# wenbowen123/iros20-6d-pose-tracking

Measured on NVIDIA H100. Metric: rgbd_pair_frames_per_sec, higher is better.
Workload: dtype bf16x3 (bf16 hi/lo split operands, 3 products/MAC, fp32 accumulate)

## Files before the change

### iros20-6d-pose-tracking_b200/csrc/conv_wgmma.cu

```cuda
#include "conv_common.h"
#include "launch.h"
#include "ptx.cuh"
#include "storage.cuh"
#include <algorithm>

namespace se3tn {
namespace {

constexpr int kThreads2 = 384;
constexpr int kPoolPitch = 68;
constexpr int kPoolStageBytes = 121 * kPoolPitch * 4;
constexpr int kPoolStageAlloc = (kPoolStageBytes + 1023) & ~1023;
constexpr int kWgRowBytes = 64 * kChunkBytes;

template <int KIND> struct KTab;
template <> struct KTab<KIND_S1> {
    static constexpr int NU = 3;
    static constexpr int kAUnit = 19 * 1024;
    __host__ __device__ static constexpr int ntaps(int) { return 3; }
    __host__ __device__ static constexpr int wtap(int u, int k) { return k * 3 + u; }
    __host__ __device__ static constexpr int amap(int) { return 0; }
    __host__ __device__ static constexpr int c1(int u) { return u - 1; }
    __host__ __device__ static constexpr int c2(int) { return -1; }
    __host__ __device__ static constexpr int rows(int) { return 11 * 13; }
};
template <> struct KTab<KIND_S2> {
    static constexpr int NU = 6;
    static constexpr int kAUnit = 19 * 1024;
    __host__ __device__ static constexpr int ntaps(int u) { return (u & 1) ? 2 : 1; }
    __host__ __device__ static constexpr int wtap(int u, int k) { return (u & 1) ? (k == 0 ? (u >> 1) : 6 + (u >> 1)) : 3 + (u >> 1); }
    __host__ __device__ static constexpr int amap(int u) { return (u & 1) * 2 + ((u >> 1) == 1 ? 0 : 1); }
    __host__ __device__ static constexpr int c1(int u) { return (u >> 1) == 0 ? -1 : 0; }
    __host__ __device__ static constexpr int c2(int u) { return (u & 1) ? -1 : 0; }
    __host__ __device__ static constexpr int rows(int u) { return (u & 1) ? 11 * 12 : 11 * 11; }
};
template <> struct KTab<KIND_STEM> {
    static constexpr int NU = 2;
    static constexpr int kAUnit = 21 * 1024;
    __host__ __device__ static constexpr int ntaps(int u) { return u == 0 ? 4 : 3; }
    __host__ __device__ static constexpr int wtap(int u, int k) { return 2 * k + u; }
    __host__ __device__ static constexpr int amap(int u) { return u; }
    __host__ __device__ static constexpr int c1(int) { return 0; }
    __host__ __device__ static constexpr int c2(int) { return 0; }
    __host__ __device__ static constexpr int rows(int u) { return u == 0 ? 11 * 14 : 11 * 13; }
};
constexpr int kRowShift = 11;

__device__ __forceinline__ float selu_fast(float x) {
    constexpr float kAlpha = 1.6732632423543772f, kScale = 1.0507009873554805f;
    return x > 0.f ? kScale * x : (kScale * kAlpha) * (__expf(x) - 1.f);
}
__device__ __forceinline__ float act_apply(float x, int act) {
    return act == ACT_RELU ? fmaxf(x, 0.f) : (act == ACT_SELU ? selu_fast(x) : x);
}

__device__ __forceinline__ unsigned long long gtimer() { unsigned long long t; asm volatile("mov.u64 %0, %%globaltimer;" : "=l"(t)); return t; }
__device__ __forceinline__ void trace_stamp(unsigned long long* tr, int slot) { if (tr) tr[blockIdx.x * 8 + slot] = gtimer(); }
__device__ __forceinline__ void trace_exit(unsigned long long* tr) {
    if (!tr) return;
    unsigned smid; asm volatile("mov.u32 %0, %%smid;" : "=r"(smid));
    tr[blockIdx.x * 8 + 7] = (gtimer() & ~0xffull) | (smid & 0xff);
}
__device__ __forceinline__ void tile_stamp(unsigned long long* tt, int tile, int k) {
    if (tt && tile < SE3TN_TRACE_TILES) tt[tile * 4 + k] = k == 3 ? (gtimer() & ~0xffull) | (blockIdx.x & 0xff) : gtimer();
}

using ptx::desc_lo;
using ptx::mk_desc;

__device__ __forceinline__ float (&acc_lo32(float (&d)[64]))[32] { return *reinterpret_cast<float (*)[32]>(&d[0]); }

struct Consumer {
    int ct, cg, cw, ew, lane, R, m;
    __device__ __forceinline__ Consumer() {
        ct = static_cast<int>(threadIdx.x) - 128; cg = ct >> 7; ew = ct >> 5; cw = ew & 3; lane = ct & 31; R = lane >> 2; m = lane & 3;
    }
    __device__ __forceinline__ bool leader() const { return (ct & 127) == 0; }
    __device__ __forceinline__ int row(int half, int h) const { return 64 * half + 16 * cw + R + 8 * h; }
};

constexpr int kProducerRegs = 40;
constexpr int kConsumerRegs = 232;
constexpr int kTurnBar = 1;
constexpr int kStageBar = 3;
constexpr int kEpiBar = 5;

template <int N> struct Ring {
    uint32_t phase = 0;
    int stage = 0;
    __device__ __forceinline__ void next() { if (++stage == N) { stage = 0; phase ^= 1; } }
    __device__ __forceinline__ void skip(int n) {
        stage += n;
        phase ^= static_cast<uint32_t>(stage / N) & 1u;
        stage %= N;
    }
    __device__ __forceinline__ uint32_t producer_parity() const { return phase ^ 1; }
    __device__ __forceinline__ uint32_t consumer_parity() const { return phase; }
};

struct Turn {
    int base, g;
    __device__ __forceinline__ void begin() const { if (g == 1) ptx::bar_arrive(base, 256); }
    __device__ __forceinline__ void wait() const { ptx::bar_sync(base + g, 256); }
    __device__ __forceinline__ void pass() const { ptx::bar_arrive(base + (g ^ 1), 256); }
    __device__ __forceinline__ bool mine(int t) const { return (t & 1) == g; }
    __device__ __forceinline__ void end(int turns) const { if (mine(turns)) wait(); }
};

template <int KIND, int N>
__device__ __forceinline__ void load_a_units(const LayerDesc& L, int ox, int oy, int cbase, int img, int c0, int c1,
                                             uint8_t* sA, uint64_t* a_full, uint64_t* a_empty, Ring<N>& ring)
{
    using KT = KTab<KIND>;
    for (int ch = c0; ch < c1; ++ch) {
#pragma unroll
        for (int u = 0; u < KT::NU; ++u) {
            ptx::mbar_wait(&a_empty[ring.stage], ring.producer_parity());
            ptx::mbar_arrive_expect_tx(&a_full[ring.stage], static_cast<uint32_t>(KT::rows(u)) * kChunkBytes);
            ptx::tma_load_4d(sA + ring.stage * KT::kAUnit, &L.amap[KT::amap(u)], &a_full[ring.stage],
                             cbase + ch * 32, ox + KT::c1(u), oy + KT::c2(u), img);
            ring.next();
        }
    }
}

template <int PREC, int N>
__device__ __forceinline__ void mma_chunk(float (&acc)[N / 2], uint32_t a_lo, uint32_t b_lo, uint32_t fresh) {
#pragma unroll
    for (int kk = 0; kk < 4; ++kk) {
        const uint64_t a = mk_desc(a_lo + 2 * kk), b = mk_desc(b_lo + 2 * kk);
        const uint32_t f = fresh | (kk ? 1u : 0u);
        if constexpr (PREC == SE3TN_PREC_TF32) {
            if constexpr (N == 64) ptx::wgmma_tf32_n64(acc, a, b, f); else ptx::wgmma_tf32_n128(acc, a, b, f);
        } else if constexpr (PREC == SE3TN_PREC_FP8) {
            static_assert(N == 128, "e4m3 MMAs only in the trunk");
            ptx::wgmma_e4m3_n128(acc, a, b, f);
        } else if constexpr (PREC == SE3TN_PREC_FP16) {
            if constexpr (N == 64) ptx::wgmma_f16_n64(acc, a, b, f); else ptx::wgmma_f16_n128(acc, a, b, f);
        } else {
            if constexpr (N == 64) ptx::wgmma_bf16_n64(acc, a, b, f); else ptx::wgmma_bf16_n128(acc, a, b, f);
        }
    }
}

template <int KIND, int PREC> struct RCfg {
    static constexpr bool POOL = (KIND == KIND_STEM);
    static constexpr int BN = 64;
    static constexpr int kStack = ((POOL ? stem_input_prec(PREC) : PREC) == SE3TN_PREC_BF16X3) ? 2 : 1;
    static constexpr int kBTile = BN * kStack * kChunkBytes;
    static constexpr int kAStages = POOL ? (PREC == SE3TN_PREC_TF32 ? 4 : 3) : (prec_2byte(PREC) ? 6 : 4);
    static constexpr int kPoolBufs = POOL ? (PREC == SE3TN_PREC_TF32 ? 2 : 1) : 0;
    static constexpr int kAcc = BN * kStack / 2;
    static constexpr int kMaxWTiles = POOL ? 7 : ((PREC == SE3TN_PREC_TF32) ? 18 : 9);
    static constexpr int kSmem = kAStages * KTab<KIND>::kAUnit + kMaxWTiles * kBTile + kPoolBufs * kPoolStageAlloc + 1024 + 512;
    static_assert(kSmem <= 232448, "shared memory budget");
};

template <int KIND, int PREC>
__device__ __forceinline__ void resident_mma_unit(float (&acc)[RCfg<KIND, PREC>::kAcc], uint32_t a_unit_lo, const uint8_t* sB,
                                                  int u, int ch, int tiles_per_tap, uint32_t& fresh)
{
    using C = RCfg<KIND, PREC>;
    using KT = KTab<KIND>;
#pragma unroll
    for (int k = 0; k < 4; ++k) {
        if (k >= KT::ntaps(u)) break;
        const uint32_t a_lo = a_unit_lo + k * kRowShift * (kChunkBytes >> 4);
        uint32_t b_lo;
        if (C::kStack == 2) b_lo = desc_lo(sB + KT::wtap(u, k) * C::kBTile) + ch * 4;
        else                b_lo = desc_lo(sB + (KT::wtap(u, k) * tiles_per_tap + ch) * C::kBTile);
        if constexpr (C::kStack == 2 && !C::POOL) {
#pragma unroll
            for (int sl = 0; sl < 2; ++sl) {
                ptx::wgmma_bf16_n128(acc, mk_desc(a_lo + 2 * sl), mk_desc(b_lo + 2 * sl), fresh | (sl ? 1u : 0u));
                ptx::wgmma_bf16_n64(acc_lo32(acc), mk_desc(a_lo + 4 + 2 * sl), mk_desc(b_lo + 2 * sl), 1u);
            }
        } else {
            mma_chunk<C::POOL ? stem_input_prec(PREC) : PREC, C::BN * C::kStack>(acc, a_lo, b_lo, fresh);
        }
        fresh = 1u;
    }
}

template <int KIND, int PREC, bool PP>
__global__ void __launch_bounds__(kThreads2, 1)
conv_resident_kernel(const __grid_constant__ ResidentParams p)
{
    constexpr int AP = resident_prec(PREC);
    static_assert(PREC != SE3TN_PREC_FP8 || KIND == KIND_S1, "e4m3 output: the 64-channel layers only");
    using C = RCfg<KIND, AP>;
    using KT = KTab<KIND>;
    constexpr bool POOL = C::POOL;
    constexpr int NH = PP ? 2 : 1;
    constexpr bool kShareStage = PP && C::kPoolBufs == 1;
    extern __shared__ uint8_t smem_raw[];
    uint8_t* smem = reinterpret_cast<uint8_t*>((reinterpret_cast<uintptr_t>(smem_raw) + 1023) & ~uintptr_t(1023));
    const LayerDesc& L = p.L;
    const int chunks = L.chunks;
    const int tiles_per_tap = (C::kStack == 2) ? 1 : chunks;
    uint8_t* sA = smem;
    uint8_t* sB = sA + C::kAStages * KT::kAUnit;
    uint8_t* sP = sB + C::kMaxWTiles * C::kBTile;
    uint64_t* bars = reinterpret_cast<uint64_t*>(sP + C::kPoolBufs * kPoolStageAlloc);
    uint64_t* a_full = bars;
    uint64_t* a_empty = a_full + C::kAStages;
    uint64_t* b_full = a_empty + C::kAStages;
    uint64_t* b_empty = b_full + KT::NU;

    ptx::grid_dep_launch();
    if (threadIdx.x == 0) trace_stamp(p.trace, 0);
    const int warp = threadIdx.x >> 5;
    const int lane = threadIdx.x & 31;
    const int tiles_img = L.tiles_x * L.tiles_y;
    const int w_begin = static_cast<int>(static_cast<long long>(blockIdx.x) * p.m_tiles / gridDim.x);
    const int w_end = static_cast<int>(static_cast<long long>(blockIdx.x + 1) * p.m_tiles / gridDim.x);
    auto img_of = [&](int tile) -> int { return p.img_first + tile / tiles_img; };
    auto wid_of = [&](int tile) -> int { return p.img_wid ? p.img_wid[img_of(tile)] : -1; };

    if (threadIdx.x == 0) {
        for (int s = 0; s < C::kAStages; ++s) { ptx::mbar_init(&a_full[s], 1); ptx::mbar_init(&a_empty[s], PP ? 1 : 2); }
        for (int u = 0; u < KT::NU; ++u) ptx::mbar_init(&b_full[u], 1);
        ptx::mbar_init(&b_empty[0], 2);
        ptx::fence_barrier_init();
        ptx::fence_proxy_async();
    }
    __syncthreads();
    if (threadIdx.x == 0) trace_stamp(p.trace, 1);

    if (warp < 4) {
        ptx::setmaxnreg_dec<kProducerRegs>();
        if (warp == 0) {
            if (lane == 0) {
                ptx::grid_dep_wait();
                Ring<C::kAStages> ring;
                for (int tile = w_begin; tile < w_end; ++tile) {
                    const int n0 = img_of(tile), r = tile % tiles_img;
                    const int ty = r / L.tiles_x, tx = r - ty * L.tiles_x;
                    load_a_units<KIND>(L, tx * p.step_x + p.off_x, ty * p.step_y + p.off_y, 0, n0, 0, chunks, sA, a_full, a_empty, ring);
                }
            }
        } else if (warp == 1) {
            if (lane == 0) {
                int cur = -2; uint32_t gen = 0;
                for (int tile = w_begin; tile < w_end; ++tile) {
                    const int wid = wid_of(tile);
                    if (wid == cur) continue;
                    if (gen) ptx::mbar_wait(&b_empty[0], (gen - 1) & 1);
                    const CUtensorMap* bm = wid < 0 ? &L.bmap : p.gbmaps + wid * kLayersPerSet + L.li;
#pragma unroll
                    for (int u = 0; u < KT::NU; ++u) {
                        ptx::mbar_arrive_expect_tx(&b_full[u], static_cast<uint32_t>(KT::ntaps(u) * tiles_per_tap) * C::kBTile);
#pragma unroll
                        for (int k = 0; k < KT::ntaps(u); ++k)
                            for (int c = 0; c < tiles_per_tap; ++c) {
                                const int wt = KT::wtap(u, k) * tiles_per_tap + c;
                                ptx::tma_load_2d(sB + wt * C::kBTile, bm, &b_full[u], wt * 32, 0);
                            }
                    }
                    cur = wid; ++gen;
                }
            }
        }
    } else {
        ptx::setmaxnreg_inc<kConsumerRegs>();
        ptx::grid_dep_wait();
        using S = Storage<AP>;
        const Consumer cs;
        const bool stamp = threadIdx.x == 128;
        const bool tstamp = cs.leader() && (PP || cs.cg == 0);
        constexpr int kEpiThreads = PP ? 128 : 256;
        const int et = PP ? (cs.ct & 127) : cs.ct;
        auto half_of = [&](int hf) { return PP ? hf : cs.cg; };
        Ring<C::kAStages> a_ring;
        int w_cur = -2; uint32_t w_gen = 0;
        const Turn turn{kTurnBar, cs.cg}, stage_turn{kStageBar, cs.cg};
        if constexpr (PP) {
            turn.begin();
            if constexpr (kShareStage) stage_turn.begin();
        }
        int it = 0;
        for (int tile = w_begin; tile < w_end; ++tile, ++it) {
            const int wid = wid_of(tile);
            const bool new_w = (wid != w_cur);
            const bool w_last = tile + 1 < w_end && wid_of(tile + 1) != wid;
            if (PP && !turn.mine(it)) {
                a_ring.skip(chunks * KT::NU);
                if (new_w) {
#pragma unroll
                    for (int u = 0; u < KT::NU; ++u) ptx::mbar_wait(&b_full[u], w_gen & 1);
                    w_cur = wid; ++w_gen;
                }
                if (w_last && cs.leader()) ptx::mbar_arrive(&b_empty[0]);
                continue;
            }
            const int n0 = img_of(tile), r = tile % tiles_img;
            const int ty = r / L.tiles_x, tx = r - ty * L.tiles_x;

            constexpr int kPreRes = (PP && C::kStack == 2) ? 1 : NH;
            size_t rpix[NH][2]; bool rvalid[NH][2]; Raw<AP, 8> rres[NH][2][2];
            auto load_res = [&](int hf) {
#pragma unroll
                for (int h = 0; h < 2; ++h) {
                    const int rw = cs.row(half_of(hf), h);
                    const int py = rw / 11, px = rw - py * 11;
                    const int y = ty * 11 + py, x = tx * 11 + px;
                    rvalid[hf][h] = (rw < 121) && (y < L.Ho) && (x < L.Wo);
                    rpix[hf][h] = (static_cast<size_t>(n0) * L.Ho + y) * L.Wo + x;
#pragma unroll
                    for (int b = 0; b < 2; ++b) {
                        rres[hf][h][b] = Raw<AP, 8>{};
                        if (L.res && rvalid[hf][h]) {
                            const uint8_t* rp = L.res + S::addr(rpix[hf][h], L.res_c, 32 * b + 8 * cs.m);
#pragma unroll
                            for (int q = 0; q < Raw<AP, 8>::kPieces; ++q) rres[hf][h][b].set(q, __ldg(Raw<AP, 8>::at(rp, q)));
                        }
                    }
                }
            };
            if constexpr (!POOL) {
#pragma unroll
                for (int hf = 0; hf < kPreRes; ++hf) load_res(hf);
            }
            float4 pb4 = make_float4(0.f, 0.f, 0.f, 0.f);
            if constexpr (POOL) pb4 = __ldg(reinterpret_cast<const float4*>((p.img_wid ? p.gbias[p.img_wid[n0] * kLayersPerSet + L.li] : L.bias) + (et & 15) * 4));

            float acc[NH][C::kAcc];
#pragma unroll
            for (int hf = 0; hf < NH; ++hf)
#pragma unroll
                for (int i = 0; i < C::kAcc; ++i) acc[hf][i] = 0.f;
            if constexpr (PP) turn.wait();
            uint32_t fresh = 0;
            int pend = -1;
            for (int ch = 0; ch < chunks; ++ch) {
#pragma unroll
                for (int u = 0; u < KT::NU; ++u) {
                    if (new_w && ch == 0) {
                        ptx::mbar_wait(&b_full[u], w_gen & 1);
                        if (it == 0 && u == 0 && stamp) trace_stamp(p.trace, 2);
                    }
                    ptx::mbar_wait(&a_full[a_ring.stage], a_ring.consumer_parity());
                    if (ch == 0 && u == 0) {
                        if (it == 0 && stamp) trace_stamp(p.trace, 3);
                        if (tstamp) tile_stamp(p.tile_trace, tile, 0);
                    }
                    ptx::wgmma_fence();
                    const uint32_t a_unit_lo = desc_lo(sA + a_ring.stage * KT::kAUnit);
#pragma unroll
                    for (int hf = 0; hf < NH; ++hf) {
                        uint32_t f = fresh;
                        resident_mma_unit<KIND, AP>(acc[hf], a_unit_lo + half_of(hf) * (kWgRowBytes >> 4), sB, u, ch, tiles_per_tap, f);
                    }
                    fresh = 1u;
                    ptx::wgmma_commit();
                    ptx::wgmma_wait<1>();
                    if (pend >= 0 && cs.leader()) ptx::mbar_arrive(&a_empty[pend]);
                    pend = a_ring.stage;
                    a_ring.next();
                }
            }
            if constexpr (PP) turn.pass();
            ptx::wgmma_wait<0>();
#pragma unroll
            for (int hf = 0; hf < NH; ++hf) ptx::wgmma_reg_fence(acc[hf]);
            if (tstamp) tile_stamp(p.tile_trace, tile, 1);
            if (cs.leader()) {
                ptx::mbar_arrive(&a_empty[pend]);
                if (w_last) ptx::mbar_arrive(&b_empty[0]);
            }
            if (new_w) { w_cur = wid; ++w_gen; }
            if (it == 0 && stamp) trace_stamp(p.trace, 5);
            if (tstamp) tile_stamp(p.tile_trace, tile, 2);

            if constexpr (!POOL) {
                float inv_out = 1.f;
                if constexpr (PREC == SE3TN_PREC_FP8) inv_out = 1.f / __ldg((p.img_wid ? p.gfp8[p.img_wid[n0]] : p.fp8) + L.q_out);
#pragma unroll
                for (int hf = 0; hf < NH; ++hf) {
                    if (hf >= kPreRes) load_res(hf);
#pragma unroll
                    for (int b = 0; b < 2; ++b) {
                        const int ch0 = 32 * b + 8 * cs.m;
                        const float* bias_base = (p.img_wid ? p.gbias[p.img_wid[n0] * kLayersPerSet + L.li] : L.bias) + ch0;
                        const float4 bA = __ldg(reinterpret_cast<const float4*>(bias_base)), bB = __ldg(reinterpret_cast<const float4*>(bias_base + 4));
                        const float bias8[8] = {bA.x, bA.y, bA.z, bA.w, bB.x, bB.y, bB.z, bB.w};
#pragma unroll
                        for (int h = 0; h < 2; ++h) {
                            if (!rvalid[hf][h]) continue;
                            float v[8];
#pragma unroll
                            for (int jj = 0; jj < 4; ++jj)
#pragma unroll
                                for (int e = 0; e < 2; ++e) {
                                    const int ri = 16 * b + 4 * jj + 2 * h + e;
                                    float a = acc[hf][ri];
                                    if constexpr (C::kStack == 2) a += acc[hf][32 + ri];
                                    v[2 * jj + e] = a + bias8[2 * jj + e];
                                }
                            if (L.res) {
                                float r[8];
                                S::decode(rres[hf][h][b], r);
#pragma unroll
                                for (int e = 0; e < 8; ++e) v[e] += r[e];
                            }
#pragma unroll
                            for (int e = 0; e < 8; ++e) v[e] = act_apply(v[e], L.act);
                            if constexpr (PREC == SE3TN_PREC_FP8) {
                                using S8 = Storage<SE3TN_PREC_FP8>;
#pragma unroll
                                for (int e = 0; e < 8; ++e) v[e] *= inv_out;
                                S8::encode(v).store(L.out + S8::addr(rpix[hf][h], L.out_c, L.out_coff + ch0));
                            } else {
                                S::encode(v).store(L.out + S::addr(rpix[hf][h], L.out_c, L.out_coff + ch0));
                            }
                        }
                    }
                }
            } else {
                float* stage = reinterpret_cast<float*>(sP + (C::kPoolBufs == 2 ? (it & 1) : 0) * kPoolStageAlloc);
                if constexpr (kShareStage) stage_turn.wait();
                else if constexpr (PP) ptx::bar_sync(kEpiBar + cs.cg, 128);
#pragma unroll
                for (int hf = 0; hf < NH; ++hf)
#pragma unroll
                    for (int h = 0; h < 2; ++h) {
                        const int rw = cs.row(half_of(hf), h);
                        if (rw >= 121) continue;
                        const int cy_l = rw / 11, cx_l = rw - cy_l * 11;
                        const int cy = ty * p.step_y + p.off_y + cy_l, cx = tx * p.step_x + p.off_x + cx_l;
                        const bool cvalid = cy >= 0 && cy < 88 && cx >= 0 && cx < 88;
                        float* srow = stage + rw * kPoolPitch + 2 * cs.m;
                        const float ninf = -3.0e38f;
#pragma unroll
                        for (int j = 0; j < 8; ++j) {
                            float a0 = acc[hf][4 * j + 2 * h], a1 = acc[hf][4 * j + 2 * h + 1];
                            if constexpr (C::kStack == 2) { a0 += acc[hf][32 + 4 * j + 2 * h]; a1 += acc[hf][32 + 4 * j + 2 * h + 1]; }
                            *reinterpret_cast<float2*>(srow + 8 * j) = cvalid ? make_float2(a0, a1) : make_float2(ninf, ninf);
                        }
                    }
                ptx::bar_sync(PP ? kEpiBar + cs.cg : kEpiBar, kEpiThreads);

                for (int v = et; v < 400; v += kEpiThreads) {
                    const int pp = v >> 4, c4 = (v & 15) * 4;
                    const int ppy = pp / 5, ppx = pp - ppy * 5;
                    const int oy = ty * 5 + ppy, ox = tx * 5 + ppx;
                    if (oy >= L.Ho || ox >= L.Wo) continue;
                    float4 mx = make_float4(-3.0e38f, -3.0e38f, -3.0e38f, -3.0e38f);
#pragma unroll
                    for (int dy = 0; dy < 3; ++dy)
#pragma unroll
                        for (int dx = 0; dx < 3; ++dx) {
                            const float4 s4 = *reinterpret_cast<const float4*>(stage + ((2 * ppy + dy) * 11 + 2 * ppx + dx) * kPoolPitch + c4);
                            mx.x = fmaxf(mx.x, s4.x); mx.y = fmaxf(mx.y, s4.y); mx.z = fmaxf(mx.z, s4.z); mx.w = fmaxf(mx.w, s4.w);
                        }
                    const float v4[4] = {selu_fast(mx.x + pb4.x), selu_fast(mx.y + pb4.y), selu_fast(mx.z + pb4.z), selu_fast(mx.w + pb4.w)};
                    S::encode(v4).store(L.out + S::addr((static_cast<size_t>(n0) * L.Ho + oy) * L.Wo + ox, L.out_c, L.out_coff + c4));
                }
                if constexpr (kShareStage) stage_turn.pass();
                else if constexpr (!PP) { if (C::kPoolBufs == 1) ptx::bar_sync(kEpiBar, 256); }
            }
            if (tstamp) tile_stamp(p.tile_trace, tile, 3);
        }
        if constexpr (PP) {
            turn.end(it);
            if constexpr (kShareStage) stage_turn.end(it);
        }
        if (stamp) { trace_stamp(p.trace, 4); trace_stamp(p.trace, 6); }
    }

    __syncthreads();
    if (threadIdx.x == 0) trace_exit(p.trace);
}

template <int PREC> struct TCfg {
    static constexpr int BN = 128;
    static constexpr int kAcc = BN / 2;
    static constexpr int kAStages = 3;
    static constexpr int kBStages = 6;
    static constexpr int kBTile = BN * kChunkBytes;
    static constexpr int kEpiPitch = 36;
    static constexpr int kEpiWarpBytes = 16 * kEpiPitch * 4 + 128;
    static constexpr int kEpiBytes = 8 * kEpiWarpBytes;
    static constexpr int kSched = 4;
    static constexpr int kAUnit = KTab<KIND_S1>::kAUnit;
    static_assert(kAUnit == KTab<KIND_S2>::kAUnit, "A ring stage size");
    static constexpr int kSmem = kAStages * kAUnit + kBStages * kBTile + ((kEpiBytes + 1023) & ~1023) + 1024 + 512;
    static_assert(kSmem <= 232448, "shared memory budget");
};
constexpr int kTaps3 = 9;

struct UnitCoord { int l, img, tx, ty, n_tile, grp, c0, c1, piece, gidx; };
__device__ __forceinline__ void unit_stamp(const TrunkParams& p, int u, int k) {
    if (p.trace && u < 2048) p.trace[256 * 8 + u * 5 + k] = k == 4 ? (gtimer() & ~0xffull) | (blockIdx.x & 0xff) : gtimer();
}

__device__ __forceinline__ int unit_layer(const TrunkParams& p, int u) {
    int l = 0;
#pragma unroll
    for (int i = 1; i < kTrunkMaxLayers; ++i) if (i < p.n_layers && u >= p.layer[i].unit_base) l = i;
    return l;
}

__device__ __forceinline__ UnitCoord decode_unit(const TrunkParams& p, int u) {
    UnitCoord c;
    c.l = unit_layer(p, u);
    const LayerDesc& L = p.layer[c.l];
    int local = u - L.unit_base;
    c.piece = 0; c.c0 = 0; c.c1 = L.chunks;
    if (p.ksplit > 1) {
        c.piece = local % p.ksplit; local /= p.ksplit;
        c.c0 = c.piece * L.chunks / p.ksplit; c.c1 = (c.piece + 1) * L.chunks / p.ksplit;
    }
    c.gidx = L.base_unit0 + local;
    const int im = local / L.units_per_image;
    int r = local - im * L.units_per_image;
    c.img = p.img_first + im;
    c.n_tile = r % L.n_tiles; r /= L.n_tiles;
    c.grp = r % L.groups; r /= L.groups;
    c.ty = r / L.tiles_x; c.tx = r - c.ty * L.tiles_x;
    return c;
}

template <int KIND, int PREC>
__device__ __forceinline__ void trunk_load_weights(const LayerDesc& L, const CUtensorMap* bm, const UnitCoord& c, uint8_t* sB,
                                                   uint64_t* b_full, uint64_t* b_empty, Ring<TCfg<PREC>::kBStages>& ring)
{
    using KT = KTab<KIND>;
    using C = TCfg<PREC>;
    const int wrow = c.grp * L.cout + c.n_tile * C::BN;
    for (int ch = c.c0; ch < c.c1; ++ch) {
#pragma unroll
        for (int u = 0; u < KT::NU; ++u) {
#pragma unroll
            for (int k = 0; k < KT::ntaps(u); ++k) {
                ptx::mbar_wait(&b_empty[ring.stage], ring.producer_parity());
                ptx::mbar_arrive_expect_tx(&b_full[ring.stage], C::kBTile);
                ptx::tma_load_2d(sB + ring.stage * C::kBTile, bm, &b_full[ring.stage], KT::wtap(u, k) * L.cin_words + ch * 32, wrow);
                ring.next();
            }
        }
    }
}

template <int KIND, int PREC>
__device__ __forceinline__ void trunk_mma_unit(float (&acc)[2][TCfg<PREC>::kAcc], const Consumer& cs, const Turn& turn, int chunks,
                                               uint8_t* sA, uint8_t* sB, uint64_t* a_full, uint64_t* a_empty, uint64_t* b_full,
                                               uint64_t* b_empty, Ring<TCfg<PREC>::kAStages>& a_ring, Ring<TCfg<PREC>::kBStages>& b_ring,
                                               unsigned long long* trace, bool first_unit, unsigned long long* ustamp)
{
    using KT = KTab<KIND>;
    using C = TCfg<PREC>;
    const bool stamp = cs.leader();
    uint32_t fresh = 0;
    int pend_b = -1, pend_a = -1;
    turn.wait();
    for (int ch = 0; ch < chunks; ++ch) {
#pragma unroll
        for (int u = 0; u < KT::NU; ++u) {
            ptx::mbar_wait(&a_full[a_ring.stage], a_ring.consumer_parity());
            if (first_unit && ch == 0 && u == 0 && stamp) trace_stamp(trace, 3);
            if (ustamp && ch == 0 && u == 0 && stamp) *ustamp = gtimer();
            const uint32_t a_unit_lo = desc_lo(sA + a_ring.stage * C::kAUnit);
#pragma unroll
            for (int k = 0; k < KT::ntaps(u); ++k) {
                ptx::mbar_wait(&b_full[b_ring.stage], b_ring.consumer_parity());
                if (first_unit && ch == 0 && u == 0 && k == 0 && stamp) trace_stamp(trace, 2);
                const uint32_t b_lo = desc_lo(sB + b_ring.stage * C::kBTile);
                ptx::wgmma_fence();
#pragma unroll
                for (int hf = 0; hf < 2; ++hf) {
                    const uint32_t a_lo = a_unit_lo + hf * (kWgRowBytes >> 4) + k * kRowShift * (kChunkBytes >> 4);
                    if constexpr (PREC == SE3TN_PREC_BF16X3) {
                        constexpr int AO[6] = {0, 2, 4, 6, 0, 2};
                        constexpr int BO[6] = {0, 2, 0, 2, 4, 6};
#pragma unroll
                        for (int i = 0; i < 6; ++i)
                            ptx::wgmma_bf16_n128(acc[hf], mk_desc(a_lo + AO[i]), mk_desc(b_lo + BO[i]), fresh | (i ? 1u : 0u));
                    } else {
                        mma_chunk<PREC, C::BN>(acc[hf], a_lo, b_lo, fresh);
                    }
                }
                ptx::wgmma_commit();
                ptx::wgmma_wait<1>();
                if (cs.leader()) {
                    if (pend_b >= 0) ptx::mbar_arrive(&b_empty[pend_b]);
                    if (pend_a >= 0) ptx::mbar_arrive(&a_empty[pend_a]);
                }
                pend_b = b_ring.stage;
                pend_a = (k + 1 == KT::ntaps(u)) ? a_ring.stage : -1;
                fresh = 1u;
                b_ring.next();
            }
            a_ring.next();
        }
    }
    turn.pass();
    ptx::wgmma_wait<0>();
    ptx::wgmma_reg_fence(acc[0]);
    ptx::wgmma_reg_fence(acc[1]);
    if (cs.leader()) {
        if (pend_b >= 0) ptx::mbar_arrive(&b_empty[pend_b]);
        if (pend_a >= 0) ptx::mbar_arrive(&a_empty[pend_a]);
    }
}

template <int PREC>
__global__ void __launch_bounds__(kThreads2, 1)
conv_trunk_kernel(const __grid_constant__ TrunkParams p)
{
    using C = TCfg<PREC>;
    constexpr int BN = C::BN;
    extern __shared__ uint8_t smem_raw[];
    uint8_t* smem = reinterpret_cast<uint8_t*>((reinterpret_cast<uintptr_t>(smem_raw) + 1023) & ~uintptr_t(1023));
    uint8_t* sA = smem;
    uint8_t* sB = sA + C::kAStages * C::kAUnit;
    uint8_t* sT = sB + C::kBStages * C::kBTile;
    uint64_t* bars = reinterpret_cast<uint64_t*>(sT + ((C::kEpiBytes + 1023) & ~1023));
    uint64_t* a_full = bars;
    uint64_t* a_empty = a_full + C::kAStages;
// ... 353 lines not shown
```

### iros20-6d-pose-tracking_b200/csrc/ptx.cuh

```cuda
#pragma once
#include <cstdint>
#include <cuda.h>

namespace ptx {

__device__ __forceinline__ uint32_t smem_u32(const void* p) {
    return static_cast<uint32_t>(__cvta_generic_to_shared(p));
}

__device__ __forceinline__ bool elect_one() {
    uint32_t pred = 0;
    asm volatile(
        "{\n\t.reg .pred P;\n\t"
        "elect.sync _|P, 0xffffffff;\n\t"
        "selp.u32 %0, 1, 0, P;\n\t}\n"
        : "=r"(pred));
    return pred != 0;
}

__device__ __forceinline__ int ld_acquire_gpu(const int* p) {
    int v;
    asm volatile("ld.acquire.gpu.global.s32 %0, [%1];" : "=r"(v) : "l"(p) : "memory");
    return v;
}
__device__ __forceinline__ void st_release_gpu(int* p, int v) {
    asm volatile("st.release.gpu.global.s32 [%0], %1;" :: "l"(p), "r"(v) : "memory");
}
__device__ __forceinline__ void grid_dep_launch() { asm volatile("griddepcontrol.launch_dependents;" ::: "memory"); }
__device__ __forceinline__ void grid_dep_wait()   { asm volatile("griddepcontrol.wait;" ::: "memory"); }

template <int N> __device__ __forceinline__ void setmaxnreg_dec() { asm volatile("setmaxnreg.dec.sync.aligned.u32 %0;" ::"n"(N)); }
template <int N> __device__ __forceinline__ void setmaxnreg_inc() { asm volatile("setmaxnreg.inc.sync.aligned.u32 %0;" ::"n"(N)); }
__device__ __forceinline__ void bar_sync(int id, int n)   { asm volatile("bar.sync %0, %1;" ::"r"(id), "r"(n) : "memory"); }
__device__ __forceinline__ void bar_arrive(int id, int n) { asm volatile("bar.arrive %0, %1;" ::"r"(id), "r"(n) : "memory"); }

__device__ __forceinline__ void mbar_init(uint64_t* bar, uint32_t count) {
    asm volatile("mbarrier.init.shared::cta.b64 [%0], %1;" ::"r"(smem_u32(bar)), "r"(count));
}
__device__ __forceinline__ void fence_barrier_init() {
    asm volatile("fence.mbarrier_init.release.cluster;" ::: "memory");
}
__device__ __forceinline__ void fence_proxy_async() {
    asm volatile("fence.proxy.async.shared::cta;" ::: "memory");
}
__device__ __forceinline__ void fence_proxy_async_all() {
    asm volatile("fence.proxy.async;" ::: "memory");
}
__device__ __forceinline__ void mbar_arrive_expect_tx(uint64_t* bar, uint32_t bytes) {
    asm volatile("mbarrier.arrive.expect_tx.shared::cta.b64 _, [%0], %1;"
                 ::"r"(smem_u32(bar)), "r"(bytes) : "memory");
}
__device__ __forceinline__ void mbar_arrive(uint64_t* bar) {
    asm volatile("mbarrier.arrive.shared::cta.b64 _, [%0];" ::"r"(smem_u32(bar)) : "memory");
}
__device__ __forceinline__ bool mbar_try_wait(uint64_t* bar, uint32_t parity) {
    uint32_t ok;
    asm volatile(
        "{\n\t.reg .pred P;\n\t"
        "mbarrier.try_wait.parity.shared::cta.b64 P, [%1], %2;\n\t"
        "selp.u32 %0, 1, 0, P;\n\t}\n"
        : "=r"(ok) : "r"(smem_u32(bar)), "r"(parity) : "memory");
    return ok != 0;
}
static __device__ __noinline__ void timeout_trap() { __trap(); }

__device__ __forceinline__ void mbar_wait(uint64_t* bar, uint32_t parity) {
    if (mbar_try_wait(bar, parity)) return;
    const long long t0 = clock64();
    while (!mbar_try_wait(bar, parity)) {
        if (clock64() - t0 > (1ll << 35)) timeout_trap();
    }
}

__device__ __forceinline__ void prefetch_tmap(const CUtensorMap* m) {
    asm volatile("prefetch.tensormap [%0];" ::"l"(reinterpret_cast<uint64_t>(m)) : "memory");
}
__device__ __forceinline__ void tma_load_2d(void* dst, const CUtensorMap* m, uint64_t* bar, int c0, int c1) {
    asm volatile(
        "cp.async.bulk.tensor.2d.shared::cluster.global.tile.mbarrier::complete_tx::bytes"
        " [%0], [%1, {%3, %4}], [%2];"
        ::"r"(smem_u32(dst)), "l"(reinterpret_cast<uint64_t>(m)), "r"(smem_u32(bar)), "r"(c0), "r"(c1)
        : "memory");
}
__device__ __forceinline__ void tma_load_4d(void* dst, const CUtensorMap* m, uint64_t* bar,
                                            int c0, int c1, int c2, int c3) {
    asm volatile(
        "cp.async.bulk.tensor.4d.shared::cluster.global.tile.mbarrier::complete_tx::bytes"
        " [%0], [%1, {%3, %4, %5, %6}], [%2];"
        ::"r"(smem_u32(dst)), "l"(reinterpret_cast<uint64_t>(m)), "r"(smem_u32(bar)),
          "r"(c0), "r"(c1), "r"(c2), "r"(c3)
        : "memory");
}

__device__ __forceinline__ void wgmma_fence()  { asm volatile("wgmma.fence.sync.aligned;" ::: "memory"); }
__device__ __forceinline__ void wgmma_commit() { asm volatile("wgmma.commit_group.sync.aligned;" ::: "memory"); }
template <int N>
__device__ __forceinline__ void wgmma_wait() { asm volatile("wgmma.wait_group.sync.aligned %0;" ::"n"(N) : "memory"); }
template <int N>
__device__ __forceinline__ void wgmma_reg_fence(float (&d)[N]) {
#pragma unroll
    for (int i = 0; i < N; ++i) asm volatile("" : "+f"(d[i])::"memory");
}

constexpr uint32_t kDescHi = (1024u >> 4) | (1u << 30);
__device__ __forceinline__ uint32_t desc_lo(const void* smem_ptr) { return ((smem_u32(smem_ptr) & 0x3FFFFu) >> 4) | (1u << 16); }
__device__ __forceinline__ uint64_t mk_desc(uint32_t lo) { return (static_cast<uint64_t>(kDescHi) << 32) | lo; }

__device__ __forceinline__ void wgmma_bf16_n64(float (&d)[32], uint64_t adesc, uint64_t bdesc, uint32_t accumulate) {
    asm volatile(
        "{\n\t.reg .pred p;\n\t"
        "setp.ne.b32 p, %34, 0;\n\t"
        "wgmma.mma_async.sync.aligned.m64n64k16.f32.bf16.bf16 {"
        "%0, %1, %2, %3, %4, %5, %6, %7, %8, %9, %10, %11, %12, %13, %14, %15, "
        "%16, %17, %18, %19, %20, %21, %22, %23, %24, %25, %26, %27, %28, %29, %30, %31"
        "}, %32, %33, p, 1, 1, 0, 0;\n\t}\n"
        : "+f"(d[0]), "+f"(d[1]), "+f"(d[2]), "+f"(d[3]), "+f"(d[4]), "+f"(d[5]), "+f"(d[6]), "+f"(d[7])
        , "+f"(d[8]), "+f"(d[9]), "+f"(d[10]), "+f"(d[11]), "+f"(d[12]), "+f"(d[13]), "+f"(d[14]), "+f"(d[15])
        , "+f"(d[16]), "+f"(d[17]), "+f"(d[18]), "+f"(d[19]), "+f"(d[20]), "+f"(d[21]), "+f"(d[22]), "+f"(d[23])
        , "+f"(d[24]), "+f"(d[25]), "+f"(d[26]), "+f"(d[27]), "+f"(d[28]), "+f"(d[29]), "+f"(d[30]), "+f"(d[31])
        : "l"(adesc), "l"(bdesc), "r"(accumulate));
}
__device__ __forceinline__ void wgmma_bf16_n128(float (&d)[64], uint64_t adesc, uint64_t bdesc, uint32_t accumulate) {
    asm volatile(
        "{\n\t.reg .pred p;\n\t"
        "setp.ne.b32 p, %66, 0;\n\t"
        "wgmma.mma_async.sync.aligned.m64n128k16.f32.bf16.bf16 {"
        "%0, %1, %2, %3, %4, %5, %6, %7, %8, %9, %10, %11, %12, %13, %14, %15, "
        "%16, %17, %18, %19, %20, %21, %22, %23, %24, %25, %26, %27, %28, %29, %30, %31, "
        "%32, %33, %34, %35, %36, %37, %38, %39, %40, %41, %42, %43, %44, %45, %46, %47, "
        "%48, %49, %50, %51, %52, %53, %54, %55, %56, %57, %58, %59, %60, %61, %62, %63"
        "}, %64, %65, p, 1, 1, 0, 0;\n\t}\n"
        : "+f"(d[0]), "+f"(d[1]), "+f"(d[2]), "+f"(d[3]), "+f"(d[4]), "+f"(d[5]), "+f"(d[6]), "+f"(d[7])
        , "+f"(d[8]), "+f"(d[9]), "+f"(d[10]), "+f"(d[11]), "+f"(d[12]), "+f"(d[13]), "+f"(d[14]), "+f"(d[15])
        , "+f"(d[16]), "+f"(d[17]), "+f"(d[18]), "+f"(d[19]), "+f"(d[20]), "+f"(d[21]), "+f"(d[22]), "+f"(d[23])
        , "+f"(d[24]), "+f"(d[25]), "+f"(d[26]), "+f"(d[27]), "+f"(d[28]), "+f"(d[29]), "+f"(d[30]), "+f"(d[31])
        , "+f"(d[32]), "+f"(d[33]), "+f"(d[34]), "+f"(d[35]), "+f"(d[36]), "+f"(d[37]), "+f"(d[38]), "+f"(d[39])
        , "+f"(d[40]), "+f"(d[41]), "+f"(d[42]), "+f"(d[43]), "+f"(d[44]), "+f"(d[45]), "+f"(d[46]), "+f"(d[47])
        , "+f"(d[48]), "+f"(d[49]), "+f"(d[50]), "+f"(d[51]), "+f"(d[52]), "+f"(d[53]), "+f"(d[54]), "+f"(d[55])
        , "+f"(d[56]), "+f"(d[57]), "+f"(d[58]), "+f"(d[59]), "+f"(d[60]), "+f"(d[61]), "+f"(d[62]), "+f"(d[63])
        : "l"(adesc), "l"(bdesc), "r"(accumulate));
}
__device__ __forceinline__ void wgmma_f16_n64(float (&d)[32], uint64_t adesc, uint64_t bdesc, uint32_t accumulate) {
    asm volatile(
        "{\n\t.reg .pred p;\n\t"
        "setp.ne.b32 p, %34, 0;\n\t"
        "wgmma.mma_async.sync.aligned.m64n64k16.f32.f16.f16 {"
        "%0, %1, %2, %3, %4, %5, %6, %7, %8, %9, %10, %11, %12, %13, %14, %15, "
        "%16, %17, %18, %19, %20, %21, %22, %23, %24, %25, %26, %27, %28, %29, %30, %31"
        "}, %32, %33, p, 1, 1, 0, 0;\n\t}\n"
        : "+f"(d[0]), "+f"(d[1]), "+f"(d[2]), "+f"(d[3]), "+f"(d[4]), "+f"(d[5]), "+f"(d[6]), "+f"(d[7])
        , "+f"(d[8]), "+f"(d[9]), "+f"(d[10]), "+f"(d[11]), "+f"(d[12]), "+f"(d[13]), "+f"(d[14]), "+f"(d[15])
        , "+f"(d[16]), "+f"(d[17]), "+f"(d[18]), "+f"(d[19]), "+f"(d[20]), "+f"(d[21]), "+f"(d[22]), "+f"(d[23])
        , "+f"(d[24]), "+f"(d[25]), "+f"(d[26]), "+f"(d[27]), "+f"(d[28]), "+f"(d[29]), "+f"(d[30]), "+f"(d[31])
        : "l"(adesc), "l"(bdesc), "r"(accumulate));
}
__device__ __forceinline__ void wgmma_f16_n128(float (&d)[64], uint64_t adesc, uint64_t bdesc, uint32_t accumulate) {
    asm volatile(
        "{\n\t.reg .pred p;\n\t"
        "setp.ne.b32 p, %66, 0;\n\t"
        "wgmma.mma_async.sync.aligned.m64n128k16.f32.f16.f16 {"
        "%0, %1, %2, %3, %4, %5, %6, %7, %8, %9, %10, %11, %12, %13, %14, %15, "
        "%16, %17, %18, %19, %20, %21, %22, %23, %24, %25, %26, %27, %28, %29, %30, %31, "
        "%32, %33, %34, %35, %36, %37, %38, %39, %40, %41, %42, %43, %44, %45, %46, %47, "
        "%48, %49, %50, %51, %52, %53, %54, %55, %56, %57, %58, %59, %60, %61, %62, %63"
        "}, %64, %65, p, 1, 1, 0, 0;\n\t}\n"
        : "+f"(d[0]), "+f"(d[1]), "+f"(d[2]), "+f"(d[3]), "+f"(d[4]), "+f"(d[5]), "+f"(d[6]), "+f"(d[7])
        , "+f"(d[8]), "+f"(d[9]), "+f"(d[10]), "+f"(d[11]), "+f"(d[12]), "+f"(d[13]), "+f"(d[14]), "+f"(d[15])
        , "+f"(d[16]), "+f"(d[17]), "+f"(d[18]), "+f"(d[19]), "+f"(d[20]), "+f"(d[21]), "+f"(d[22]), "+f"(d[23])
        , "+f"(d[24]), "+f"(d[25]), "+f"(d[26]), "+f"(d[27]), "+f"(d[28]), "+f"(d[29]), "+f"(d[30]), "+f"(d[31])
        , "+f"(d[32]), "+f"(d[33]), "+f"(d[34]), "+f"(d[35]), "+f"(d[36]), "+f"(d[37]), "+f"(d[38]), "+f"(d[39])
        , "+f"(d[40]), "+f"(d[41]), "+f"(d[42]), "+f"(d[43]), "+f"(d[44]), "+f"(d[45]), "+f"(d[46]), "+f"(d[47])
        , "+f"(d[48]), "+f"(d[49]), "+f"(d[50]), "+f"(d[51]), "+f"(d[52]), "+f"(d[53]), "+f"(d[54]), "+f"(d[55])
        , "+f"(d[56]), "+f"(d[57]), "+f"(d[58]), "+f"(d[59]), "+f"(d[60]), "+f"(d[61]), "+f"(d[62]), "+f"(d[63])
        : "l"(adesc), "l"(bdesc), "r"(accumulate));
}
__device__ __forceinline__ void wgmma_tf32_n64(float (&d)[32], uint64_t adesc, uint64_t bdesc, uint32_t accumulate) {
    asm volatile(
        "{\n\t.reg .pred p;\n\t"
        "setp.ne.b32 p, %34, 0;\n\t"
        "wgmma.mma_async.sync.aligned.m64n64k8.f32.tf32.tf32 {"
        "%0, %1, %2, %3, %4, %5, %6, %7, %8, %9, %10, %11, %12, %13, %14, %15, "
        "%16, %17, %18, %19, %20, %21, %22, %23, %24, %25, %26, %27, %28, %29, %30, %31"
        "}, %32, %33, p, 1, 1;\n\t}\n"
        : "+f"(d[0]), "+f"(d[1]), "+f"(d[2]), "+f"(d[3]), "+f"(d[4]), "+f"(d[5]), "+f"(d[6]), "+f"(d[7])
        , "+f"(d[8]), "+f"(d[9]), "+f"(d[10]), "+f"(d[11]), "+f"(d[12]), "+f"(d[13]), "+f"(d[14]), "+f"(d[15])
        , "+f"(d[16]), "+f"(d[17]), "+f"(d[18]), "+f"(d[19]), "+f"(d[20]), "+f"(d[21]), "+f"(d[22]), "+f"(d[23])
        , "+f"(d[24]), "+f"(d[25]), "+f"(d[26]), "+f"(d[27]), "+f"(d[28]), "+f"(d[29]), "+f"(d[30]), "+f"(d[31])
        : "l"(adesc), "l"(bdesc), "r"(accumulate));
}
__device__ __forceinline__ void wgmma_tf32_n128(float (&d)[64], uint64_t adesc, uint64_t bdesc, uint32_t accumulate) {
    asm volatile(
        "{\n\t.reg .pred p;\n\t"
        "setp.ne.b32 p, %66, 0;\n\t"
        "wgmma.mma_async.sync.aligned.m64n128k8.f32.tf32.tf32 {"
        "%0, %1, %2, %3, %4, %5, %6, %7, %8, %9, %10, %11, %12, %13, %14, %15, "
        "%16, %17, %18, %19, %20, %21, %22, %23, %24, %25, %26, %27, %28, %29, %30, %31, "
        "%32, %33, %34, %35, %36, %37, %38, %39, %40, %41, %42, %43, %44, %45, %46, %47, "
        "%48, %49, %50, %51, %52, %53, %54, %55, %56, %57, %58, %59, %60, %61, %62, %63"
        "}, %64, %65, p, 1, 1;\n\t}\n"
        : "+f"(d[0]), "+f"(d[1]), "+f"(d[2]), "+f"(d[3]), "+f"(d[4]), "+f"(d[5]), "+f"(d[6]), "+f"(d[7])
        , "+f"(d[8]), "+f"(d[9]), "+f"(d[10]), "+f"(d[11]), "+f"(d[12]), "+f"(d[13]), "+f"(d[14]), "+f"(d[15])
        , "+f"(d[16]), "+f"(d[17]), "+f"(d[18]), "+f"(d[19]), "+f"(d[20]), "+f"(d[21]), "+f"(d[22]), "+f"(d[23])
        , "+f"(d[24]), "+f"(d[25]), "+f"(d[26]), "+f"(d[27]), "+f"(d[28]), "+f"(d[29]), "+f"(d[30]), "+f"(d[31])
        , "+f"(d[32]), "+f"(d[33]), "+f"(d[34]), "+f"(d[35]), "+f"(d[36]), "+f"(d[37]), "+f"(d[38]), "+f"(d[39])
        , "+f"(d[40]), "+f"(d[41]), "+f"(d[42]), "+f"(d[43]), "+f"(d[44]), "+f"(d[45]), "+f"(d[46]), "+f"(d[47])
        , "+f"(d[48]), "+f"(d[49]), "+f"(d[50]), "+f"(d[51]), "+f"(d[52]), "+f"(d[53]), "+f"(d[54]), "+f"(d[55])
        , "+f"(d[56]), "+f"(d[57]), "+f"(d[58]), "+f"(d[59]), "+f"(d[60]), "+f"(d[61]), "+f"(d[62]), "+f"(d[63])
        : "l"(adesc), "l"(bdesc), "r"(accumulate));
}

__device__ __forceinline__ void wgmma_e4m3_n128(float (&d)[64], uint64_t adesc, uint64_t bdesc, uint32_t accumulate) {
    asm volatile(
        "{\n\t.reg .pred p;\n\t"
        "setp.ne.b32 p, %66, 0;\n\t"
        "wgmma.mma_async.sync.aligned.m64n128k32.f32.e4m3.e4m3 {"
        "%0, %1, %2, %3, %4, %5, %6, %7, %8, %9, %10, %11, %12, %13, %14, %15, "
        "%16, %17, %18, %19, %20, %21, %22, %23, %24, %25, %26, %27, %28, %29, %30, %31, "
        "%32, %33, %34, %35, %36, %37, %38, %39, %40, %41, %42, %43, %44, %45, %46, %47, "
        "%48, %49, %50, %51, %52, %53, %54, %55, %56, %57, %58, %59, %60, %61, %62, %63"
        "}, %64, %65, p, 1, 1;\n\t}\n"
        : "+f"(d[0]), "+f"(d[1]), "+f"(d[2]), "+f"(d[3]), "+f"(d[4]), "+f"(d[5]), "+f"(d[6]), "+f"(d[7])
        , "+f"(d[8]), "+f"(d[9]), "+f"(d[10]), "+f"(d[11]), "+f"(d[12]), "+f"(d[13]), "+f"(d[14]), "+f"(d[15])
        , "+f"(d[16]), "+f"(d[17]), "+f"(d[18]), "+f"(d[19]), "+f"(d[20]), "+f"(d[21]), "+f"(d[22]), "+f"(d[23])
        , "+f"(d[24]), "+f"(d[25]), "+f"(d[26]), "+f"(d[27]), "+f"(d[28]), "+f"(d[29]), "+f"(d[30]), "+f"(d[31])
        , "+f"(d[32]), "+f"(d[33]), "+f"(d[34]), "+f"(d[35]), "+f"(d[36]), "+f"(d[37]), "+f"(d[38]), "+f"(d[39])
        , "+f"(d[40]), "+f"(d[41]), "+f"(d[42]), "+f"(d[43]), "+f"(d[44]), "+f"(d[45]), "+f"(d[46]), "+f"(d[47])
        , "+f"(d[48]), "+f"(d[49]), "+f"(d[50]), "+f"(d[51]), "+f"(d[52]), "+f"(d[53]), "+f"(d[54]), "+f"(d[55])
        , "+f"(d[56]), "+f"(d[57]), "+f"(d[58]), "+f"(d[59]), "+f"(d[60]), "+f"(d[61]), "+f"(d[62]), "+f"(d[63])
        : "l"(adesc), "l"(bdesc), "r"(accumulate));
}

__device__ __forceinline__ float to_tf32(float x) {
    uint32_t r;
    asm("cvt.rna.tf32.f32 %0, %1;" : "=r"(r) : "f"(x));
    return __uint_as_float(r);
// ... 4 lines not shown
```

Baseline: 36170.

## Double-buffer stem pool stage, prefetch residuals to L2, restructure pooled epilogue

For BF16x3 the stem kernel now keeps two pool staging buffers and drops to two A stages, which removes the shared-stage turn barrier between the two consumer groups. The producer warp issues bulk L2 prefetches for the residual rows that are loaded late in the epilogue. The 3x3/2 max-pool epilogue becomes a column-wise sliding max in which 80 threads reuse row maxima. Weight-id and bias lookups are carried ahead instead of recomputed through img_wid. The trade-off is fewer A pipeline stages for the stem and lower epilogue thread parallelism.

```diff
diff --git a/iros20-6d-pose-tracking_b200/csrc/conv_wgmma.cu b/iros20-6d-pose-tracking_b200/csrc/conv_wgmma.cu
--- a/iros20-6d-pose-tracking_b200/csrc/conv_wgmma.cu
+++ b/iros20-6d-pose-tracking_b200/csrc/conv_wgmma.cu
@@ -82,8 +82,7 @@
 constexpr int kProducerRegs = 40;
 constexpr int kConsumerRegs = 232;
 constexpr int kTurnBar = 1;
-constexpr int kStageBar = 3;
-constexpr int kEpiBar = 5;
+constexpr int kEpiBar = 3;
 
 template <int N> struct Ring {
     uint32_t phase = 0;
@@ -148,8 +147,8 @@
     static constexpr int BN = 64;
     static constexpr int kStack = ((POOL ? stem_input_prec(PREC) : PREC) == SE3TN_PREC_BF16X3) ? 2 : 1;
     static constexpr int kBTile = BN * kStack * kChunkBytes;
-    static constexpr int kAStages = POOL ? (PREC == SE3TN_PREC_TF32 ? 4 : 3) : (prec_2byte(PREC) ? 6 : 4);
-    static constexpr int kPoolBufs = POOL ? (PREC == SE3TN_PREC_TF32 ? 2 : 1) : 0;
+    static constexpr int kAStages = POOL ? (kStack == 2 ? 2 : 4) : (prec_2byte(PREC) ? 6 : 4);
+    static constexpr int kPoolBufs = POOL ? 2 : 0;
     static constexpr int kAcc = BN * kStack / 2;
     static constexpr int kMaxWTiles = POOL ? 7 : ((PREC == SE3TN_PREC_TF32) ? 18 : 9);
     static constexpr int kSmem = kAStages * KTab<KIND>::kAUnit + kMaxWTiles * kBTile + kPoolBufs * kPoolStageAlloc + 1024 + 512;
@@ -192,7 +191,7 @@
     using KT = KTab<KIND>;
     constexpr bool POOL = C::POOL;
     constexpr int NH = PP ? 2 : 1;
-    constexpr bool kShareStage = PP && C::kPoolBufs == 1;
+    constexpr int kPreRes = (PP && C::kStack == 2) ? 1 : NH;
     extern __shared__ uint8_t smem_raw[];
     uint8_t* smem = reinterpret_cast<uint8_t*>((reinterpret_cast<uintptr_t>(smem_raw) + 1023) & ~uintptr_t(1023));
     const LayerDesc& L = p.L;
@@ -236,6 +235,16 @@
                 for (int tile = w_begin; tile < w_end; ++tile) {
                     const int n0 = img_of(tile), r = tile % tiles_img;
                     const int ty = r / L.tiles_x, tx = r - ty * L.tiles_x;
+                    if constexpr (!POOL && kPreRes < NH) {
+                        if (L.res) {
+                            const int x0 = tx * 11, xn = min(11, L.Wo - x0);
+                            for (int py = 64 / 11; py < 11 && ty * 11 + py < L.Ho; ++py) {
+                                const size_t pix = (static_cast<size_t>(n0) * L.Ho + ty * 11 + py) * L.Wo + x0;
+                                ptx::prefetch_l2_bulk(L.res + Storage<AP>::addr(pix, L.res_c, 0),
+                                                      static_cast<uint32_t>(((xn - 1) * L.res_c + 64) * Storage<AP>::kBytes));
+                            }
+                        }
+                    }
                     load_a_units<KIND>(L, tx * p.step_x + p.off_x, ty * p.step_y + p.off_y, 0, n0, 0, chunks, sA, a_full, a_empty, ring);
                 }
             }
@@ -273,16 +282,16 @@
         auto half_of = [&](int hf) { return PP ? hf : cs.cg; };
         Ring<C::kAStages> a_ring;
         int w_cur = -2; uint32_t w_gen = 0;
-        const Turn turn{kTurnBar, cs.cg}, stage_turn{kStageBar, cs.cg};
-        if constexpr (PP) {
-            turn.begin();
-            if constexpr (kShareStage) stage_turn.begin();
-        }
+        const Turn turn{kTurnBar, cs.cg};
+        if constexpr (PP) turn.begin();
+        int wid_a = wid_of(w_begin), wid_b = w_begin + 1 < w_end ? wid_of(w_begin + 1) : -2;
         int it = 0;
         for (int tile = w_begin; tile < w_end; ++tile, ++it) {
-            const int wid = wid_of(tile);
+            const int wid = wid_a, wid_n = wid_b;
+            wid_a = wid_b;
+            wid_b = tile + 2 < w_end ? wid_of(tile + 2) : -2;
             const bool new_w = (wid != w_cur);
-            const bool w_last = tile + 1 < w_end && wid_of(tile + 1) != wid;
+            const bool w_last = tile + 1 < w_end && wid_n != wid;
             if (PP && !turn.mine(it)) {
                 a_ring.skip(chunks * KT::NU);
                 if (new_w) {
@@ -296,7 +305,6 @@
             const int n0 = img_of(tile), r = tile % tiles_img;
             const int ty = r / L.tiles_x, tx = r - ty * L.tiles_x;
 
-            constexpr int kPreRes = (PP && C::kStack == 2) ? 1 : NH;
             size_t rpix[NH][2]; bool rvalid[NH][2]; Raw<AP, 8> rres[NH][2][2];
             auto load_res = [&](int hf) {
 #pragma unroll
@@ -321,8 +329,7 @@
 #pragma unroll
                 for (int hf = 0; hf < kPreRes; ++hf) load_res(hf);
             }
-            float4 pb4 = make_float4(0.f, 0.f, 0.f, 0.f);
-            if constexpr (POOL) pb4 = __ldg(reinterpret_cast<const float4*>((p.img_wid ? p.gbias[p.img_wid[n0] * kLayersPerSet + L.li] : L.bias) + (et & 15) * 4));
+            const float* bias_set = wid < 0 ? L.bias : p.gbias[wid * kLayersPerSet + L.li];
 
             float acc[NH][C::kAcc];
 #pragma unroll
@@ -374,14 +381,14 @@
 
             if constexpr (!POOL) {
                 float inv_out = 1.f;
-                if constexpr (PREC == SE3TN_PREC_FP8) inv_out = 1.f / __ldg((p.img_wid ? p.gfp8[p.img_wid[n0]] : p.fp8) + L.q_out);
+                if constexpr (PREC == SE3TN_PREC_FP8) inv_out = 1.f / __ldg((wid < 0 ? p.fp8 : p.gfp8[wid]) + L.q_out);
 #pragma unroll
                 for (int hf = 0; hf < NH; ++hf) {
                     if (hf >= kPreRes) load_res(hf);
 #pragma unroll
                     for (int b = 0; b < 2; ++b) {
                         const int ch0 = 32 * b + 8 * cs.m;
-                        const float* bias_base = (p.img_wid ? p.gbias[p.img_wid[n0] * kLayersPerSet + L.li] : L.bias) + ch0;
+                        const float* bias_base = bias_set + ch0;
                         const float4 bA = __ldg(reinterpret_cast<const float4*>(bias_base)), bB = __ldg(reinterpret_cast<const float4*>(bias_base + 4));
                         const float bias8[8] = {bA.x, bA.y, bA.z, bA.w, bB.x, bB.y, bB.z, bB.w};
 #pragma unroll
@@ -417,9 +424,9 @@
                     }
                 }
             } else {
-                float* stage = reinterpret_cast<float*>(sP + (C::kPoolBufs == 2 ? (it & 1) : 0) * kPoolStageAlloc);
-                if constexpr (kShareStage) stage_turn.wait();
-                else if constexpr (PP) ptx::bar_sync(kEpiBar + cs.cg, 128);
+                float* stage = reinterpret_cast<float*>(sP + (it & 1) * kPoolStageAlloc);
+                const float4 pb4 = __ldg(reinterpret_cast<const float4*>(bias_set + (et & 15) * 4));
+                if constexpr (PP) ptx::bar_sync(kEpiBar + cs.cg, 128);
 #pragma unroll
                 for (int hf = 0; hf < NH; ++hf)
 #pragma unroll
@@ -440,31 +447,36 @@
                     }
                 ptx::bar_sync(PP ? kEpiBar + cs.cg : kEpiBar, kEpiThreads);
 
-                for (int v = et; v < 400; v += kEpiThreads) {
-                    const int pp = v >> 4, c4 = (v & 15) * 4;
-                    const int ppy = pp / 5, ppx = pp - ppy * 5;
-                    const int oy = ty * 5 + ppy, ox = tx * 5 + ppx;
-                    if (oy >= L.Ho || ox >= L.Wo) continue;
-                    float4 mx = make_float4(-3.0e38f, -3.0e38f, -3.0e38f, -3.0e38f);
-#pragma unroll
-                    for (int dy = 0; dy < 3; ++dy)
-#pragma unroll
-                        for (int dx = 0; dx < 3; ++dx) {
-                            const float4 s4 = *reinterpret_cast<const float4*>(stage + ((2 * ppy + dy) * 11 + 2 * ppx + dx) * kPoolPitch + c4);
-                            mx.x = fmaxf(mx.x, s4.x); mx.y = fmaxf(mx.y, s4.y); mx.z = fmaxf(mx.z, s4.z); mx.w = fmaxf(mx.w, s4.w);
-                        }
-                    const float v4[4] = {selu_fast(mx.x + pb4.x), selu_fast(mx.y + pb4.y), selu_fast(mx.z + pb4.z), selu_fast(mx.w + pb4.w)};
-                    S::encode(v4).store(L.out + S::addr((static_cast<size_t>(n0) * L.Ho + oy) * L.Wo + ox, L.out_c, L.out_coff + c4));
-                }
-                if constexpr (kShareStage) stage_turn.pass();
-                else if constexpr (!PP) { if (C::kPoolBufs == 1) ptx::bar_sync(kEpiBar, 256); }
+                if (et < 80) {
+                    const int ppx = et >> 4, c4 = (et & 15) * 4;
+                    const int ox = tx * 5 + ppx;
+                    if (ox < L.Wo) {
+                        const float* col = stage + 2 * ppx * kPoolPitch + c4;
+                        auto row_max = [&](int cy_l) {
+                            const float* s = col + cy_l * 11 * kPoolPitch;
+                            const float4 a = *reinterpret_cast<const float4*>(s), b = *reinterpret_cast<const float4*>(s + kPoolPitch),
+                                         c = *reinterpret_cast<const float4*>(s + 2 * kPoolPitch);
+                            return make_float4(fmaxf(fmaxf(a.x, b.x), c.x), fmaxf(fmaxf(a.y, b.y), c.y),
+                                               fmaxf(fmaxf(a.z, b.z), c.z), fmaxf(fmaxf(a.w, b.w), c.w));
+                        };
+                        float4 top = row_max(0);
+#pragma unroll
+                        for (int ppy = 0; ppy < 5; ++ppy) {
+                            const float4 mid = row_max(2 * ppy + 1), bot = row_max(2 * ppy + 2);
+                            const float4 mx = make_float4(fmaxf(fmaxf(top.x, mid.x), bot.x), fmaxf(fmaxf(top.y, mid.y), bot.y),
+                                                          fmaxf(fmaxf(top.z, mid.z), bot.z), fmaxf(fmaxf(top.w, mid.w), bot.w));
+                            top = bot;
+                            const int oy = ty * 5 + ppy;
+                            if (oy >= L.Ho) continue;
+                            const float v4[4] = {selu_fast(mx.x + pb4.x), selu_fast(mx.y + pb4.y), selu_fast(mx.z + pb4.z), selu_fast(mx.w + pb4.w)};
+                            S::encode(v4).store(L.out + S::addr((static_cast<size_t>(n0) * L.Ho + oy) * L.Wo + ox, L.out_c, L.out_coff + c4));
+                        }
+                    }
+                }
             }
             if (tstamp) tile_stamp(p.tile_trace, tile, 3);
         }
-        if constexpr (PP) {
-            turn.end(it);
-            if constexpr (kShareStage) stage_turn.end(it);
-        }
+        if constexpr (PP) turn.end(it);
         if (stamp) { trace_stamp(p.trace, 4); trace_stamp(p.trace, 6); }
     }
 
diff --git a/iros20-6d-pose-tracking_b200/csrc/ptx.cuh b/iros20-6d-pose-tracking_b200/csrc/ptx.cuh
--- a/iros20-6d-pose-tracking_b200/csrc/ptx.cuh
+++ b/iros20-6d-pose-tracking_b200/csrc/ptx.cuh
@@ -81,6 +81,9 @@
         " [%0], [%1, {%3, %4}], [%2];"
         ::"r"(smem_u32(dst)), "l"(reinterpret_cast<uint64_t>(m)), "r"(smem_u32(bar)), "r"(c0), "r"(c1)
         : "memory");
+}
+__device__ __forceinline__ void prefetch_l2_bulk(const void* p, uint32_t bytes) {
+    asm volatile("cp.async.bulk.prefetch.L2.global [%0], %1;" ::"l"(reinterpret_cast<uint64_t>(p)), "r"(bytes) : "memory");
 }
 __device__ __forceinline__ void tma_load_4d(void* dst, const CUtensorMap* m, uint64_t* bar,
                                             int c0, int c1, int c2, int c3) {
```

Result: no change. 36270, median of 6 (+0.3%).
